# sair-lab/localization

Hardware: AMD Instinct MI355X
Metric: localization updates/sec (8-anchor UWB, batch=65k) (higher is better)
Workload: dtype f64

## Files before the change

include/localization_amd.h:

```cpp
#ifndef LOCALIZATION_AMD_H
#define LOCALIZATION_AMD_H

#include <stddef.h>
#include <stdint.h>

#ifdef __cplusplus
extern "C" {
#endif

#define LOC_ABI_VERSION 4

typedef enum loc_status {
    LOC_OK = 0,
    LOC_ERR_INVALID = -1,
    LOC_ERR_NO_DEVICE = -2,
    LOC_ERR_HIP = -3,
    LOC_ERR_UNKNOWN_NODE = -4,
    LOC_ERR_UNSUPPORTED = -5,
    LOC_ERR_SINGULAR = -6
} loc_status;

enum { LOC_JAC_ANALYTIC = 0, LOC_JAC_NUMERIC_G2O = 1 };

const char* loc_last_error(void);
int32_t loc_abi_version(void);
int32_t loc_device_count(void);

typedef struct loc_shard {
    int32_t rank, world;
    int32_t device;
    int32_t reserved;
    int64_t lo, hi;
} loc_shard;
int loc_shard_bounds(int64_t total, int32_t rank, int32_t world, int64_t* lo, int64_t* hi);
int loc_shard_plan(int64_t total, int32_t world, int32_t devices_per_node, loc_shard* out);

typedef struct loc_snapshot loc_snapshot;

typedef struct loc_snapshot_params {
    int32_t maximum_iteration;
    double distance_outlier;
    int32_t gate_warmup_epochs;
    int32_t jacobian;
    int32_t lanes_per_instance;
    int32_t block_threads;
} loc_snapshot_params;

void loc_snapshot_default_params(loc_snapshot_params* p);

int loc_snapshot_create(loc_snapshot** out, int32_t device, int64_t batch, int32_t n_anchors,
                        const double* anchors_xyz_host, const loc_snapshot_params* params);
int loc_snapshot_destroy(loc_snapshot* s);

int64_t loc_snapshot_batch(const loc_snapshot* s);
int32_t loc_snapshot_anchor_groups(const loc_snapshot* s);
int32_t loc_snapshot_lanes_per_instance(const loc_snapshot* s);
size_t loc_snapshot_range_floats(const loc_snapshot* s, int32_t epochs);

int loc_snapshot_set_positions(loc_snapshot* s, const double* pos_soa_host);
int loc_snapshot_get_positions(loc_snapshot* s, double* pos_soa_host);
void* loc_snapshot_positions_device(loc_snapshot* s);
int64_t loc_snapshot_epochs_done(const loc_snapshot* s);
int loc_snapshot_set_epochs_done(loc_snapshot* s, int64_t epochs);

int loc_snapshot_pack_ranges_host(const loc_snapshot* s, int32_t epochs, const float* src_kmb, float* dst_tiles,
                                  float pad_value);

int loc_snapshot_solve_device(loc_snapshot* s, int32_t epochs, const float* dist_dev, const float* err_dev,
                              double* out_pos_dev, double* out_chi2_dev, uint8_t* out_trials_dev,
                              void* hip_stream);

int loc_snapshot_solve_host(loc_snapshot* s, int32_t epochs, const float* dist_tiles_host,
                            const float* err_tiles_host, double* out_pos_host, double* out_chi2_host,
                            uint8_t* out_trials_host);

int loc_snapshot_solve_host_kmb(loc_snapshot* s, int32_t epochs, const float* dist_kmb_host, const float* err_kmb_host,
                                double* out_pos_host, double* out_chi2_host, uint8_t* out_trials_host);

// ... 178 lines not shown
```

localization_amd/_lib.py:

```python
import ctypes as C
import os

_HERE = os.path.dirname(os.path.abspath(__file__))
_SO = os.environ.get("LOCALIZATION_AMD_LIB") or os.path.join(_HERE, "liblocalization_amd.so")
_LIB = None

LOC_OK = 0
LOC_ERR_NO_DEVICE = -2
JAC_ANALYTIC = 0
JAC_NUMERIC_G2O = 1


class LocalizationAmdError(RuntimeError):
    def __init__(self, code, msg):
        super().__init__(f"localization_amd error {code}: {msg}")
        self.code = code


class SnapshotParams(C.Structure):
    _fields_ = [("maximum_iteration", C.c_int32), ("distance_outlier", C.c_double), ("gate_warmup_epochs", C.c_int32), ("jacobian", C.c_int32),
                ("lanes_per_instance", C.c_int32), ("block_threads", C.c_int32)]


class FusionParams(C.Structure):
    _fields_ = [("maximum_iteration", C.c_int32), ("distance_outlier", C.c_double), ("gate_warmup_epochs", C.c_int32),
                ("antenna_offset", C.c_double * 3), ("block_threads", C.c_int32), ("jacobian", C.c_int32)]


def library_path():
    return _SO


EXPORTED_SYMBOLS = [
    "loc_last_error", "loc_abi_version", "loc_device_count", "loc_shard_bounds", "loc_shard_plan",
    "loc_snapshot_default_params", "loc_snapshot_create", "loc_snapshot_destroy", "loc_snapshot_batch",
    "loc_snapshot_anchor_groups", "loc_snapshot_lanes_per_instance", "loc_snapshot_range_floats",
    "loc_snapshot_set_positions", "loc_snapshot_get_positions", "loc_snapshot_positions_device",
    "loc_snapshot_epochs_done", "loc_snapshot_set_epochs_done",
    "loc_snapshot_pack_ranges_host", "loc_snapshot_solve_device", "loc_snapshot_solve_host",
    "loc_snapshot_solve_host_kmb", "loc_snapshot_solve_device_cov", "loc_snapshot_solve_host_kmb_cov", "loc_host_alloc", "loc_host_free",
    "loc_snapshot_timing_begin", "loc_snapshot_timing_end",
    "loc_window_create", "loc_window_destroy", "loc_window_set_anchors", "loc_window_lds_bytes", "loc_window_solve_host",
    "loc_window_last_kernel_ms", "loc_window_set_endpoint1_offsets", "loc_window_set_prior_information", "loc_window_set_jacobian", "loc_window_set_ordering", "loc_window_set_chain_threshold", "loc_window_last_kernel_kind", "loc_window_set_option", "loc_window_last_host_timing", "loc_window_upload",
    "loc_window_solve_resident", "loc_window_download", "loc_window_poses_device", "loc_window_result_device",
    "loc_window_timing_begin", "loc_window_timing_end",
    "loc_window_covariance_host", "loc_window_covariance_resident", "loc_window_last_covariance_ms", "loc_window_covariance_plan",
    "loc_window_marginal_prior_host", "loc_window_joint_covariance_host", "loc_window_joint_covariance_resident", "loc_window_joint_covariance_plan",
    "loc_window_slide_resident", "loc_window_slide_resident_dev", "loc_window_download_tables",
    "loc_node_default_config", "loc_node_create", "loc_node_destroy", "loc_node_add_range", "loc_node_add_imu",
    "loc_node_add_pose", "loc_node_add_twist", "loc_node_add_lidar", "loc_node_add_rl_range", "loc_node_solve", "loc_node_get_path",
    "loc_node_number_measurements", "loc_node_last_timing", "loc_node_last_kernel_kind", "loc_node_flush_tail", "loc_node_set_deferred", "loc_node_solve_pending", "loc_nodes_solve_batch",
    "loc_nodes_release_batch_cache",
    "loc_fusion_default_params", "loc_fusion_create", "loc_fusion_destroy", "loc_fusion_set_poses", "loc_fusion_get_poses",
    "loc_fusion_solve_device", "loc_fusion_solve_host", "loc_fusion_solve_host_kmb", "loc_fusion_last_kernel_ms", "loc_fusion_timing_begin", "loc_fusion_timing_end",
# ... 198 lines not shown
```

localization_amd/csrc/capi.cpp:

```cpp
#include <algorithm>
#include <cmath>
#include <cstdio>
#include <cstring>
#include <new>
#include <string>
#include <vector>

#include "capi_host.h"
#include "snapshot_kernel.h"

static thread_local std::string g_last_error;

int locamd_fail(int code, const char* what) {
    g_last_error = what ? what : "";
    return code;
}
int locamd_fail_hip(hipError_t e, const char* where) {
    g_last_error = std::string(where) + ": " + hipGetErrorString(e);
    return LOC_ERR_HIP;
}

struct loc_snapshot {
    int device = 0;
    long long B = 0;
// ... 24 lines not shown
}

int loc_shard_bounds(int64_t total, int32_t rank, int32_t world, int64_t* lo, int64_t* hi) {
    if (total < 0 || world <= 0 || rank < 0 || rank >= world || !lo || !hi) return locamd_fail(LOC_ERR_INVALID, "loc_shard_bounds arguments");
    const int64_t per = (total + world - 1) / world;
    const int64_t a = rank * per < total ? rank * per : total;
    *lo = a;
    *hi = a + per < total ? a + per : total;
    return LOC_OK;
}

int loc_shard_plan(int64_t total, int32_t world, int32_t devices_per_node, loc_shard* out) {
    if (total < 0 || world <= 0 || !out) return locamd_fail(LOC_ERR_INVALID, "loc_shard_plan arguments");
    if (devices_per_node <= 0) {
        devices_per_node = loc_device_count();
        if (devices_per_node <= 0) return locamd_fail(LOC_ERR_NO_DEVICE, "no HIP device visible: pass devices_per_node explicitly");
    }
    for (int32_t r = 0; r < world; ++r) {
        out[r].rank = r; out[r].world = world; out[r].device = r % devices_per_node; out[r].reserved = 0;
        const int rc = loc_shard_bounds(total, r, world, &out[r].lo, &out[r].hi);
        if (rc != LOC_OK) return rc;
    }
    return LOC_OK;
}

void loc_snapshot_default_params(loc_snapshot_params* p) {
    if (!p) return;
    p->maximum_iteration = 20;
    p->distance_outlier = 1.0;
    p->gate_warmup_epochs = 1;
    p->jacobian = LOC_JAC_NUMERIC_G2O;
    p->lanes_per_instance = 0;
    p->block_threads = 0;
}

int loc_snapshot_create(loc_snapshot** out, int32_t device, int64_t batch, int32_t n_anchors,
                        const double* anchors_xyz_host, const loc_snapshot_params* params) {
    if (!out) return locamd_fail(LOC_ERR_INVALID, "out is NULL");
    *out = nullptr;
    if (batch <= 0 || n_anchors <= 0 || !anchors_xyz_host) return locamd_fail(LOC_ERR_INVALID, "batch/anchors");
    int ndev = 0;
    if (hipGetDeviceCount(&ndev) != hipSuccess || ndev <= 0)
        return locamd_fail(LOC_ERR_NO_DEVICE, "no HIP device visible: localization_amd has no CPU fallback");
    if (device < 0 || device >= ndev) return locamd_fail(LOC_ERR_INVALID, "device index out of range");
    loc_snapshot_params prm;
    if (params) prm = *params; else loc_snapshot_default_params(&prm);
    if (prm.jacobian != LOC_JAC_ANALYTIC && prm.jacobian != LOC_JAC_NUMERIC_G2O) return locamd_fail(LOC_ERR_INVALID, "jacobian mode");
    const int M4 = (n_anchors + 3) / 4;
    const int M_PAD = 4 * M4;
    if (M_PAD > 16) return locamd_fail(LOC_ERR_UNSUPPORTED, "more than 16 anchors per tag");
    int lpi = prm.lanes_per_instance;
    if (lpi == 0) lpi = (M_PAD == 16) ? 2 : 1;
    if (!locamd::snapshot_supported(M_PAD, lpi)) return locamd_fail(LOC_ERR_UNSUPPORTED, "lanes_per_instance for this anchor count");
    if (prm.block_threads == 0) prm.block_threads = 256;
    if (prm.gate_warmup_epochs < 0) return locamd_fail(LOC_ERR_INVALID, "gate_warmup_epochs");
    if (prm.block_threads % 64 || prm.block_threads > 256 || prm.block_threads < 64) return locamd_fail(LOC_ERR_INVALID, "block_threads");

    LOC_HIP(hipSetDevice(device));
    loc_snapshot* s = new (std::nothrow) loc_snapshot();
    if (!s) return locamd_fail(LOC_ERR_INVALID, "out of host memory");
    s->device = device; s->B = batch; s->M = n_anchors; s->M4 = M4; s->M_PAD = M_PAD; s->lpi = lpi; s->prm = prm;
    std::vector<double> anch((size_t)M_PAD * 3, 0.0);
    std::memcpy(anch.data(), anchors_xyz_host, sizeof(double) * 3 * (size_t)n_anchors);
    hipError_t e;
    if ((e = hipMalloc((void**)&s->d_anchors, anch.size() * sizeof(double))) != hipSuccess ||
        (e = hipMalloc((void**)&s->d_pos, sizeof(double) * 3 * (size_t)batch)) != hipSuccess ||
        (e = hipMemcpy(s->d_anchors, anch.data(), anch.size() * sizeof(double), hipMemcpyHostToDevice)) != hipSuccess ||
        (e = hipMemset(s->d_pos, 0, sizeof(double) * 3 * (size_t)batch)) != hipSuccess ||
        (e = hipStreamCreateWithFlags(&s->own_stream, hipStreamNonBlocking)) != hipSuccess) {
        loc_snapshot_destroy(s);
        return locamd_fail_hip(e, "loc_snapshot_create");
    }
    *out = s;
    return LOC_OK;
}

static int ensure_staging(loc_snapshot* s, int32_t epochs) {
    const size_t nf = loc_snapshot_range_floats(s, epochs), KB = (size_t)epochs * (size_t)s->B;
    LOC_HIP(locamd::grow_buffers(s->staged_epochs, (size_t)epochs, {{s->d_dist, nf * sizeof(float)}, {s->d_err, nf * sizeof(float)},
            {s->d_out_pos, sizeof(double) * 3 * KB}, {s->d_out_chi2, sizeof(double) * KB}, {s->d_out_trials, KB}}));
    return LOC_OK;
}

int loc_snapshot_destroy(loc_snapshot* s) {
    if (!s) return LOC_OK;
    (void)hipSetDevice(s->device);
    s->pipe.destroy();
    s->timer.destroy();
// ... 37 lines not shown
    if (!s || !src || !dst || epochs <= 0) return locamd_fail(LOC_ERR_INVALID, "pack_ranges");
    const size_t B = (size_t)s->B;
    for (int k = 0; k < epochs; ++k)
        for (int g = 0; g < s->M4; ++g)
            for (int j = 0; j < 4; ++j) {
                const int m = 4 * g + j;
                float* d = dst + (((size_t)k * s->M4 + g) * B) * 4 + j;
                if (m < s->M) {
                    const float* sp = src + ((size_t)k * s->M + m) * B;
                    for (size_t b = 0; b < B; ++b) d[4 * b] = sp[b];
                } else {
                    for (size_t b = 0; b < B; ++b) d[4 * b] = pad_value;
                }
            }
    return LOC_OK;
}

}

static int solve_device(loc_snapshot* s, int32_t epochs, const float* dist_dev, const float* err_dev, double* out_pos_dev,
                        double* out_chi2_dev, uint8_t* out_trials_dev, double* cov, int32_t* cov_mask, int32_t* cov_status, void* hip_stream) {
    if (epochs <= 0 || !dist_dev || !err_dev || !out_pos_dev || !out_chi2_dev) return locamd_fail(LOC_ERR_INVALID, "solve arguments");
    if (((uintptr_t)dist_dev | (uintptr_t)err_dev) & 15u) return locamd_fail(LOC_ERR_INVALID, "range tiles must be 16-byte aligned");
    LOC_HIP(hipSetDevice(s->device));
    hipStream_t st = hip_stream ? (hipStream_t)hip_stream : s->own_stream;
    locamd::SnapshotArgs a;
    a.dist = dist_dev; a.err = err_dev; a.pos = s->d_pos; a.out_pos = out_pos_dev; a.out_chi2 = out_chi2_dev;
    a.out_trials = out_trials_dev; a.anchors = s->d_anchors; a.B = s->B; a.K = epochs; a.M4 = s->M4;
    a.iterations = s->prm.maximum_iteration; a.gate = s->prm.distance_outlier;
    {
        long long left = (long long)s->prm.gate_warmup_epochs - s->epochs_done;
        a.gate_from_epoch = left > 0 ? (int)(left > epochs ? epochs : left) : 0;
    }
    LOC_HIP(s->timer.start(st));
    hipError_t e;
    if (!cov) {
        e = locamd::launch_snapshot(a, s->M_PAD, s->lpi, s->prm.jacobian, s->prm.block_threads, st);
    } else {
        locamd::SnapshotCovArgs ca;
        static_cast<locamd::SnapshotArgs&>(ca) = a;
        ca.out_cov = cov; ca.out_cov_mask = cov_mask; ca.out_cov_status = cov_status;
        e = locamd::launch_snapshot_cov(ca, s->M_PAD, s->lpi, s->prm.jacobian, s->prm.block_threads, st);
    }
    if (e != hipSuccess) return locamd_fail_hip(e, "launch_snapshot");
    LOC_HIP(s->timer.stop(st));
    s->epochs_done += epochs;
    return LOC_OK;
}

extern "C" {

int loc_snapshot_solve_device(loc_snapshot* s, int32_t epochs, const float* dist_dev, const float* err_dev,
                              double* out_pos_dev, double* out_chi2_dev, uint8_t* out_trials_dev, void* hip_stream) {
    if (!s) return locamd_fail(LOC_ERR_INVALID, "null handle");
    return solve_device(s, epochs, dist_dev, err_dev, out_pos_dev, out_chi2_dev, out_trials_dev, nullptr, nullptr, nullptr, hip_stream);
}

int loc_snapshot_solve_device_cov(loc_snapshot* s, int32_t epochs, const float* dist_dev, const float* err_dev,
                                  double* out_pos_dev, double* out_chi2_dev, uint8_t* out_trials_dev,
                                  double* out_cov_dev, int32_t* out_cov_mask_dev, int32_t* out_cov_status_dev, void* hip_stream) {
    if (!s) return locamd_fail(LOC_ERR_INVALID, "null handle");
    if (!out_cov_dev || !out_cov_mask_dev || !out_cov_status_dev) return locamd_fail(LOC_ERR_INVALID, "covariance outputs: all three are required");
    return solve_device(s, epochs, dist_dev, err_dev, out_pos_dev, out_chi2_dev, out_trials_dev, out_cov_dev, out_cov_mask_dev,
                        out_cov_status_dev, hip_stream);
}

int loc_snapshot_solve_host(loc_snapshot* s, int32_t epochs, const float* dist_h, const float* err_h,
                            double* out_pos_h, double* out_chi2_h, uint8_t* out_trials_h) {
    if (!s) return locamd_fail(LOC_ERR_INVALID, "null handle");
    if (epochs <= 0 || !dist_h || !err_h || !out_pos_h || !out_chi2_h) return locamd_fail(LOC_ERR_INVALID, "solve arguments");
    LOC_HIP(hipSetDevice(s->device));
    const size_t nf = loc_snapshot_range_floats(s, epochs);
    const size_t B = (size_t)s->B;
    if (int rc = ensure_staging(s, epochs)) return rc;
    LOC_HIP(hipMemcpyAsync(s->d_dist, dist_h, nf * sizeof(float), hipMemcpyHostToDevice, s->own_stream));
// ... 71 lines not shown
```

localization_amd/csrc/snapshot_kernel.h:

```cpp
#pragma once
#include <hip/hip_runtime.h>
#include <stdint.h>

namespace locamd {

struct SnapshotArgs {
    const float* dist;
    const float* err;
    double* pos;
    double* out_pos;
    double* out_chi2;
    uint8_t* out_trials;
    const double* anchors;
    long long B;
    int K;
    int M4;
    int iterations;
    double gate;
    int gate_from_epoch;
};

struct SnapshotCovArgs : SnapshotArgs {
    double* out_cov;
    int32_t* out_cov_mask;
    int32_t* out_cov_status;
};

hipError_t launch_snapshot(const SnapshotArgs& a, int m_pad, int lpi, int jac, int block_threads, hipStream_t stream);
hipError_t launch_snapshot_cov(const SnapshotCovArgs& a, int m_pad, int lpi, int jac, int block_threads, hipStream_t stream);
bool snapshot_supported(int m_pad, int lpi);
hipError_t launch_pack_kmb(const float* src_kmb, float* dst_tiles, long long B, int M, int M4, int K, float pad, hipStream_t stream);

}
```

localization_amd/csrc/snapshot_kernel.hip:

```cpp
#include "snapshot_kernel.h"
#include "device_math.h"
#include "lm_damping.h"
#include "cov_device.h"

#include <float.h>
#include <math.h>

#include <type_traits>

namespace locamd {

namespace {

template <int CTRL>
__device__ __forceinline__ double dpp_move(double v) {
    int lo = __double2loint(v), hi = __double2hiint(v);
    lo = __builtin_amdgcn_update_dpp(0, lo, CTRL, 0xF, 0xF, false);
    hi = __builtin_amdgcn_update_dpp(0, hi, CTRL, 0xF, 0xF, false);
    return __hiloint2double(hi, lo);
}
constexpr int DPP_QUAD_XOR1 = 0xB1;
constexpr int DPP_QUAD_XOR2 = 0x4E;
constexpr int DPP_ROW_HALF_MIRROR = 0x141;

template <int LPI>
__device__ __forceinline__ double group_sum(double v) {
    if constexpr (LPI >= 2) v += dpp_move<DPP_QUAD_XOR1>(v);
    if constexpr (LPI >= 4) v += dpp_move<DPP_QUAD_XOR2>(v);
    if constexpr (LPI >= 8) v += dpp_move<DPP_ROW_HALF_MIRROR>(v);
    return v;
}
template <int LPI>
__device__ __forceinline__ double group_prod(double v) {
    if constexpr (LPI >= 2) v *= dpp_move<DPP_QUAD_XOR1>(v);
    if constexpr (LPI >= 4) v *= dpp_move<DPP_QUAD_XOR2>(v);
    if constexpr (LPI >= 8) v *= dpp_move<DPP_ROW_HALF_MIRROR>(v);
    return v;
}

struct System {
    double h00, h01, h02, h11, h12, h22;
    double b0, b1, b2;
    double rchi;
    double chi;
};

#pragma clang fp contract(off)
__device__ __forceinline__ double range_norm_plain(double dx, double dy, double dz) {
    return sqrt_ieee_unscaled(dx * dx + dy * dy + dz * dz);
}
__device__ __forceinline__ double range_sq_plain(double dx, double dy, double dz) { return dx * dx + dy * dy + dz * dz; }
#pragma clang fp contract(fast)

template <int LPI, int APL, int JAC>
__device__ __forceinline__ System evaluate(const double px, const double py, const double pz,
                                           const double (&ax)[APL], const double (&ay)[APL], const double (&az)[APL],
                                           const double (&d)[APL], double (&w)[APL], const double gate) {
    System s = {0, 0, 0, 0, 0, 0, 0, 0, 0, 0, 0};
    double prod = 1.0;
    int kexp = 0;
#pragma unroll
    for (int j = 0; j < APL; ++j) {
        const double dx = px - ax[j], dy = py - ay[j], dz = pz - az[j];
        double n, jx, jy, jz;
        if constexpr (JAC == 0) {
            const double n2 = fmax(dx * dx + dy * dy + dz * dz, 1e-300);
            double inv;
            sqrt_and_rsqrt_fast(n2, n, inv);
            jx = -dx * inv; jy = -dy * inv; jz = -dz * inv;
        } else {
            constexpr double delta = 1e-9;
            constexpr double scalar = 1.0 / (2 * delta);
            const double x0 = range_sq_plain(dx, dy, dz);
            double h0, c0;
            n = sqrt_ieee_unscaled_raw(x0, h0, c0);
            const double xp = (px + delta) - ax[j], xm = (px - delta) - ax[j];
            const double yp = (py + delta) - ay[j], ym = (py - delta) - ay[j];
            const double zp = (pz + delta) - az[j], zm = (pz - delta) - az[j];
            if (x0 >= 1e-5 && x0 < 1e300) {
                jx = scalar * ((d[j] - sqrt_ieee_near_c(range_sq_plain(xp, dy, dz), n, h0, c0)) - (d[j] - sqrt_ieee_near_c(range_sq_plain(xm, dy, dz), n, h0, c0)));
                jy = scalar * ((d[j] - sqrt_ieee_near_c(range_sq_plain(dx, yp, dz), n, h0, c0)) - (d[j] - sqrt_ieee_near_c(range_sq_plain(dx, ym, dz), n, h0, c0)));
                jz = scalar * ((d[j] - sqrt_ieee_near_c(range_sq_plain(dx, dy, zp), n, h0, c0)) - (d[j] - sqrt_ieee_near_c(range_sq_plain(dx, dy, zm), n, h0, c0)));
            } else {
                n = (x0 == 0.0 || x0 == __builtin_inf()) ? x0 : n;
                jx = scalar * ((d[j] - range_norm_plain(xp, dy, dz)) - (d[j] - range_norm_plain(xm, dy, dz)));
                jy = scalar * ((d[j] - range_norm_plain(dx, yp, dz)) - (d[j] - range_norm_plain(dx, ym, dz)));
                jz = scalar * ((d[j] - range_norm_plain(dx, dy, zp)) - (d[j] - range_norm_plain(dx, dy, zm)));
            }
        }
        const double e = d[j] - n;
// ... 61 lines not shown
    } else if constexpr (APL == 2) {
        const long long idx = ((k * a.M4 + m0 / 4) * B + inst) * 2 + (m0 % 4) / 2;
        const float2 dv = reinterpret_cast<const float2*>(a.dist)[idx];
        const float2 sv = reinterpret_cast<const float2*>(a.err)[idx];
        df[0] = dv.x; df[1] = dv.y; sf[0] = sv.x; sf[1] = sv.y;
    } else {
        static_assert(APL == 1 || APL == 2 || APL % 4 == 0, "anchors per lane");
        const long long idx = ((k * a.M4 + m0 / 4) * B + inst) * 4 + (m0 % 4);
        df[0] = a.dist[idx]; sf[0] = a.err[idx];
    }
}
template <int APL>
__device__ __forceinline__ void ingest(const float (&df)[APL], const float (&sf)[APL], double (&d)[APL], double (&w)[APL]) {
#pragma unroll
    for (int j = 0; j < APL; ++j) {
        const double dd = (double)df[j], ss = (double)sf[j];
        const bool valid = (ss > 0.0) && (ss < DBL_MAX) && (fabs(dd) < DBL_MAX);
        const double cov = valid ? ss * ss : 1.0;
        const double mask = valid ? 1.0 : 0.0;
        d[j] = valid ? dd : 0.0;
        w[j] = fast_rcp(cov) * mask;
    }
}

template <int APL> struct SnapshotLds {
    static constexpr int NEXT_BYTES = APL * 256 * 16;
    static constexpr int RAW_BYTES = (APL % 4 == 0) ? (2 * (APL / 4) * 256 * 16) : 0;
    static constexpr int BYTES = NEXT_BYTES + RAW_BYTES;
};

typedef __attribute__((address_space(3))) void* lds_void_ptr;
typedef const __attribute__((address_space(1))) void* glb_void_ptr;

template <int LPI, int APL, int JAC, bool COV>
__global__ void __launch_bounds__(256) snapshot_lm_kernel(const std::conditional_t<COV, SnapshotCovArgs, SnapshotArgs> a) {
    __shared__ __attribute__((aligned(16))) char lds_bytes[SnapshotLds<APL>::BYTES];
    double2* const s_next = reinterpret_cast<double2*>(lds_bytes);
    float4* const s_raw = reinterpret_cast<float4*>(lds_bytes + SnapshotLds<APL>::NEXT_BYTES);
    const int tib = threadIdx.x;
    const long long tid = (long long)blockIdx.x * blockDim.x + tib;
    const long long inst = tid / LPI;
    const int g = (int)(tid % LPI);
    const long long B = a.B;
    const int K = a.K;
    const bool live = (inst < B) && K > 0;
    const long long ld_inst = live ? inst : 0;
    bool exhausted = !live;

    double ax[APL], ay[APL], az[APL];
    const int m0 = g * APL;
#pragma unroll
    for (int j = 0; j < APL; ++j) {
        ax[j] = a.anchors[(m0 + j) * 3 + 0];
        ay[j] = a.anchors[(m0 + j) * 3 + 1];
        az[j] = a.anchors[(m0 + j) * 3 + 2];
    }

    auto put_next = [&](const double (&dd)[APL], const double (&ww)[APL]) {
#pragma unroll
        for (int j = 0; j < APL; ++j) s_next[j * 256 + tib] = make_double2(dd[j], ww[j]);
    };
    auto take_next = [&](double (&dd)[APL], double (&ww)[APL]) {
        typedef double v2f64 __attribute__((ext_vector_type(2)));
        const unsigned addr = (unsigned)(unsigned long long)(s_next + tib);
        v2f64 v[APL];
#pragma unroll
        for (int j = 0; j < APL; ++j) asm volatile("ds_read_b128 %0, %1 offset:%2" : "=v"(v[j]) : "v"(addr), "n"(j * 4096));
        if constexpr (APL == 8) {
            asm volatile("s_waitcnt lgkmcnt(0)" : "+v"(v[0]), "+v"(v[1]), "+v"(v[2]), "+v"(v[3]), "+v"(v[4]), "+v"(v[5]), "+v"(v[6]), "+v"(v[7]) :: "memory");
        } else {
#pragma unroll
            for (int j = 0; j < APL; ++j) asm volatile("s_waitcnt lgkmcnt(0)" : "+v"(v[j]) :: "memory");
        }
#pragma unroll
        for (int j = 0; j < APL; ++j) { dd[j] = v[j].x; ww[j] = v[j].y; }
    };
    auto prefetch = [&](int ke) {
        if constexpr (APL % 4 == 0) {
            const int wave_base = (tib / 64) * 64;
#pragma unroll
            for (int q4 = 0; q4 < APL / 4; ++q4) {
                const long long idx = ((long long)ke * a.M4 + (m0 / 4 + q4)) * B + ld_inst;
                __builtin_amdgcn_global_load_lds((glb_void_ptr)(reinterpret_cast<const float4*>(a.dist) + idx),
                                                 (lds_void_ptr)(s_raw + q4 * 256 + wave_base), 16, 0, 0);
                __builtin_amdgcn_global_load_lds((glb_void_ptr)(reinterpret_cast<const float4*>(a.err) + idx),
                                                 (lds_void_ptr)(s_raw + (APL / 4 + q4) * 256 + wave_base), 16, 0, 0);
            }
        }
// ... 17 lines not shown

    double px = 0, py = 0, pz = 0;
    double d[APL], w[APL];
    if (live) { px = a.pos[0 * B + inst]; py = a.pos[1 * B + inst]; pz = a.pos[2 * B + inst]; }
    {
        float df0[APL], sf0[APL];
        load_epoch<APL>(a, 0, m0, ld_inst, df0, sf0);
        ingest<APL>(df0, sf0, d, w);
        if (K > 1) {
            double dn[APL], wn[APL];
            load_epoch<APL>(a, 1, m0, ld_inst, df0, sf0);
            ingest<APL>(df0, sf0, dn, wn);
            put_next(dn, wn);
        }
        if (K > 2) prefetch(2);
    }
    asm volatile("" : "+v"(px), "+v"(py), "+v"(pz));

    System cur = {1, 0, 0, 1, 0, 1, 0, 0, 0, 0, 0};
    double cur_chi = 0, last_chi = 0, lambda = 1.0, ni = 2.0;
    int c = 0;
    int k = 0;
    int it = 0, q = 0, trials = 0;
    bool init = true;
    bool waiting = false;

    while (__any(!exhausted)) {
        const bool active = !exhausted && !waiting;
        double x0, x1, x2;
        const bool ok2 = solve3(cur, lambda, x0, x1, x2) && !init;
        if (!ok2) { x0 = 0.0; x1 = 0.0; x2 = 0.0; }
        const double tx = px + x0, ty = py + x1, tz = pz + x2;
        const bool gate_now = active && init && (a.gate > 0.0) && (k >= a.gate_from_epoch);
        const System tr = evaluate<LPI, APL, JAC>(tx, ty, tz, ax, ay, az, d, w, gate_now ? a.gate : DBL_MAX);

        const bool first = active && init;
        const bool lm = active && !init;
        const double temp_chi = ok2 ? tr.rchi : DBL_MAX;
        double scale = x0 * __builtin_fma(lambda, x0, cur.b0) + x1 * __builtin_fma(lambda, x1, cur.b1) +
                       x2 * __builtin_fma(lambda, x2, cur.b2);
        scale += lm_scale_eps;
        const double rho = (cur_chi - temp_chi) * fast_rcp(scale);
        const bool accept = lm && (rho > 0.0) && (fabs(temp_chi) < DBL_MAX) && ok2;
        if (first || accept) {
            cur = tr;
            cur_chi = tr.rchi;
            px = tx; py = ty; pz = tz;
        }
        const double lam_acc = lm_lambda_accepted(lambda, rho);
        const double lam_first = lm_tau * fmax(fabs(tr.h00), fmax(fabs(tr.h11), fabs(tr.h22)));
        lambda = first ? lam_first : (accept ? lam_acc : (lm ? lambda * ni : lambda));
        ni = (first || accept) ? 2.0 : (lm ? ni * 2.0 : ni);
        last_chi = active ? tr.chi : last_chi;
        trials = first ? 0 : trials + (lm ? 1 : 0);
        q = first ? 0 : q + (lm ? 1 : 0);
        const bool end_iter = lm && !((rho < 0.0) && (q < lm_max_trials));
        it = first ? 0 : it + (end_iter ? 1 : 0);
        const bool finished = (first && ((a.iterations <= 0) || !((tr.h00 + tr.h11 + tr.h22) > 0.0))) ||
                              (end_iter && ((q == lm_max_trials) || (rho == 0.0) || (it >= a.iterations)));
        q = end_iter ? 0 : q;
        init = active ? false : init;

        if (__any(finished)) {
            if (finished) {
                if (g == 0) {
                    a.out_pos[((long long)k * 3 + 0) * B + inst] = px;
                    a.out_pos[((long long)k * 3 + 1) * B + inst] = py;
// ... 12 lines not shown
                }
                if (k + 1 >= K) {
                    exhausted = true;
                    if (g == 0) { a.pos[0 * B + inst] = px; a.pos[1 * B + inst] = py; a.pos[2 * B + inst] = pz; }
                } else if (k == c) {
                    take_next(d, w);
                    k = c + 1;
                    init = true;
                } else {
                    waiting = true;
                }
            }
        }
        if (!__any(!exhausted && k == c)) {
            ++c;
            if (c + 1 < K) {
                double dn[APL], wn[APL];
                consume(c + 1, dn, wn);
                put_next(dn, wn);
                asm volatile("" ::: "memory");
                if (c + 2 < K) prefetch(c + 2);
                if (waiting) {
#pragma unroll
                    for (int j = 0; j < APL; ++j) { d[j] = dn[j]; w[j] = wn[j]; }
                    k = c + 1;
                    init = true;
                    waiting = false;
                }
            }
        }
    }
}

template <int LPI, int APL, int JAC, bool COV, class Args>
hipError_t launch_one(const Args& a, int block_threads, hipStream_t stream) {
    const long long lanes = a.B * LPI;
    const long long blocks = (lanes + block_threads - 1) / block_threads;
    if (blocks <= 0 || blocks > 0x7fffffffLL) return hipErrorInvalidValue;
    hipLaunchKernelGGL((snapshot_lm_kernel<LPI, APL, JAC, COV>), dim3((unsigned)blocks), dim3((unsigned)block_threads), 0, stream, a);
    return hipGetLastError();
}

template <int LPI, int APL, bool COV, class Args>
hipError_t launch_jac(const Args& a, int jac, int block_threads, hipStream_t stream) {
    return jac == 0 ? launch_one<LPI, APL, 0, COV>(a, block_threads, stream) : launch_one<LPI, APL, 1, COV>(a, block_threads, stream);
}

template <bool COV, class Args>
hipError_t launch_mapping(const Args& a, int m_pad, int lpi, int jac, int block_threads, hipStream_t stream) {
    if (!snapshot_supported(m_pad, lpi)) return hipErrorInvalidValue;
    if (block_threads <= 0) block_threads = 256;
    if (block_threads % 64 || block_threads > 256) return hipErrorInvalidValue;
    switch (m_pad * 100 + lpi) {
        case 401: return launch_jac<1, 4, COV>(a, jac, block_threads, stream);
        case 402: return launch_jac<2, 2, COV>(a, jac, block_threads, stream);
        case 404: return launch_jac<4, 1, COV>(a, jac, block_threads, stream);
        case 801: return launch_jac<1, 8, COV>(a, jac, block_threads, stream);
        case 802: return launch_jac<2, 4, COV>(a, jac, block_threads, stream);
        case 804: return launch_jac<4, 2, COV>(a, jac, block_threads, stream);
        case 808: return launch_jac<8, 1, COV>(a, jac, block_threads, stream);
        case 1201: return launch_jac<1, 12, COV>(a, jac, block_threads, stream);
        case 1601: return launch_jac<1, 16, COV>(a, jac, block_threads, stream);
        case 1602: return launch_jac<2, 8, COV>(a, jac, block_threads, stream);
        case 1604: return launch_jac<4, 4, COV>(a, jac, block_threads, stream);
        case 1608: return launch_jac<8, 2, COV>(a, jac, block_threads, stream);
        default: return hipErrorInvalidValue;
    }
}

}

namespace {
__global__ void __launch_bounds__(256) pack_kmb_kernel(const float* __restrict__ src, float4* __restrict__ dst, long long B, int M, int M4,
                                                       long long total, float pad) {
    const long long i = (long long)blockIdx.x * 256 + threadIdx.x;
    if (i >= total) return;
    const long long b = i % B, kg = i / B;
    const int g = (int)(kg % M4);
    const long long k = kg / M4;
    const float* row = src + (k * M + 4 * g) * B + b;
    float4 v;
    v.x = 4 * g + 0 < M ? row[0] : pad;
    v.y = 4 * g + 1 < M ? row[B] : pad;
    v.z = 4 * g + 2 < M ? row[2 * B] : pad;
    v.w = 4 * g + 3 < M ? row[3 * B] : pad;
    dst[i] = v;
}
}

hipError_t launch_pack_kmb(const float* src_kmb, float* dst_tiles, long long B, int M, int M4, int K, float pad, hipStream_t stream) {
    const long long total = (long long)K * M4 * B;
    if (total <= 0 || M <= 0 || M > 4 * M4) return hipErrorInvalidValue;
    const long long blocks = (total + 255) / 256;
    if (blocks > 0x7fffffffLL) return hipErrorInvalidValue;
    hipLaunchKernelGGL(pack_kmb_kernel, dim3((unsigned)blocks), dim3(256), 0, stream, src_kmb, reinterpret_cast<float4*>(dst_tiles), B, M, M4, total, pad);
    return hipGetLastError();
}

bool snapshot_supported(int m_pad, int lpi) {
    if (lpi != 1 && lpi != 2 && lpi != 4 && lpi != 8) return false;
    if (m_pad != 4 && m_pad != 8 && m_pad != 12 && m_pad != 16) return false;
    if (m_pad % lpi) return false;
    const int apl = m_pad / lpi;
    if (!(apl == 1 || apl == 2 || apl % 4 == 0)) return false;
    if (m_pad == 12 && lpi != 1) return false;
    return true;
}

hipError_t launch_snapshot(const SnapshotArgs& a, int m_pad, int lpi, int jac, int block_threads, hipStream_t stream) {
    return launch_mapping<false>(a, m_pad, lpi, jac, block_threads, stream);
}

hipError_t launch_snapshot_cov(const SnapshotCovArgs& a, int m_pad, int lpi, int jac, int block_threads, hipStream_t stream) {
    if (!a.out_cov || !a.out_cov_mask || !a.out_cov_status) return hipErrorInvalidValue;
    return launch_mapping<true>(a, m_pad, lpi, jac, block_threads, stream);
}

}
```

localization_amd/snapshot.py:

```python
import ctypes as C

import numpy as np

from . import _lib
from ._lib import SnapshotParams, check, lib


def pack_ranges(x_kmb, pad_value=0.0):
    x = np.ascontiguousarray(x_kmb, dtype=np.float32)
    K, M, B = x.shape
    M4 = (M + 3) // 4
    out = np.full((K, M4 * 4, B), pad_value, dtype=np.float32)
    out[:, :M, :] = x
    return np.ascontiguousarray(out.reshape(K, M4, 4, B).transpose(0, 1, 3, 2))


def unpack_ranges(tiles, M):
    t = np.asarray(tiles)
    K, M4, B, _ = t.shape
    return np.ascontiguousarray(t.transpose(0, 1, 3, 2).reshape(K, M4 * 4, B)[:, :M, :])


class SnapshotSolver(_lib.EpochSolver):
    _prefix = "loc_snapshot"

    def __init__(self, anchors, batch, maximum_iteration=10, distance_outlier=1.0, jacobian="numeric",
                 lanes_per_instance=0, block_threads=0, device=0, gate_warmup_epochs=1):
        import torch
        self.torch = torch
        L = lib()
        if L.loc_device_count() <= 0 or not torch.cuda.is_available():
            raise _lib.LocalizationAmdError(_lib.LOC_ERR_NO_DEVICE,
                                            "no HIP device visible: localization_amd has no CPU fallback")
        anchors = np.ascontiguousarray(anchors, dtype=np.float64)
        assert anchors.ndim == 2 and anchors.shape[1] == 3
        self.M = anchors.shape[0]
        self.B = int(batch)
        self.device = int(device)
        self.dev = torch.device("cuda", self.device)
        prm = SnapshotParams()
        L.loc_snapshot_default_params(C.byref(prm))
        prm.maximum_iteration = int(maximum_iteration)
        prm.distance_outlier = float(distance_outlier)
        prm.gate_warmup_epochs = int(gate_warmup_epochs)
        prm.jacobian = {"analytic": _lib.JAC_ANALYTIC, "numeric": _lib.JAC_NUMERIC_G2O,
                        "numeric_g2o": _lib.JAC_NUMERIC_G2O}[jacobian]
        prm.lanes_per_instance = int(lanes_per_instance)
        prm.block_threads = int(block_threads)
        h = C.c_void_p()
        check(L.loc_snapshot_create(C.byref(h), self.device, self.B, self.M,
                                    anchors.ctypes.data_as(C.POINTER(C.c_double)), C.byref(prm)))
        self.h = h
        self.L = L
        self.M4 = L.loc_snapshot_anchor_groups(h)
        self.lanes_per_instance = L.loc_snapshot_lanes_per_instance(h)

    def set_positions(self, pos_3b):
        p = np.ascontiguousarray(pos_3b, dtype=np.float64)
        assert p.shape == (3, self.B)
        check(self.L.loc_snapshot_set_positions(self.h, p.ctypes.data_as(C.POINTER(C.c_double))))

    def get_positions(self):
        p = np.zeros((3, self.B), dtype=np.float64)
        check(self.L.loc_snapshot_get_positions(self.h, p.ctypes.data_as(C.POINTER(C.c_double))))
        return p

    def to_device_tiles(self, x_kmb, pad_value=0.0):
        return self.torch.from_numpy(pack_ranges(x_kmb, pad_value)).to(self.dev)

    def alloc_outputs(self, K, trials=True, covariance=False):
        return self._device_outputs(K, 3, 6, trials, covariance)

    def solve_device(self, dist_tiles, err_tiles, out_pos, out_chi2, out_trials=None, out_cov=None, out_cov_mask=None, out_cov_status=None):
        t = self.torch
        K = dist_tiles.shape[0]
        assert tuple(dist_tiles.shape) == (K, self.M4, self.B, 4) and dist_tiles.dtype == t.float32
        assert tuple(err_tiles.shape) == tuple(dist_tiles.shape) and err_tiles.dtype == t.float32
        assert dist_tiles.is_contiguous() and err_tiles.is_contiguous()
        assert tuple(out_pos.shape) == (K, 3, self.B) and out_pos.dtype == t.float64 and out_pos.is_contiguous()
        assert tuple(out_chi2.shape) == (K, self.B) and out_chi2.dtype == t.float64 and out_chi2.is_contiguous()
        if out_trials is not None:
# ... 34 lines not shown
```

Measured before the change: 1.996 billion.

## Add cooperative wave tail that spreads per-edge work of few active tags across lanes

Adds a cooperative evaluation path for the 8-anchor, one-lane-per-tag kernel. When a wavefront has at most 8 still-active tags, those tags publish their state to LDS, each of the 64 lanes computes one (tag, edge) term, and the owning lane reduces the terms back. The goal is to cut the divergent long tail where a few unconverged tags keep a whole wave busy running serial 8-edge numeric Jacobians. In exchange it adds LDS per wave, a ballot plus wave barriers on every iteration, and extra code that may raise register pressure. It is on by default for the numeric Jacobian.

Result: no change. 1.997 billion, median of 4 (+0.1%).

```diff
diff --git a/include/localization_amd.h b/include/localization_amd.h
--- a/include/localization_amd.h
+++ b/include/localization_amd.h
@@ -44,6 +44,7 @@
     int32_t jacobian;
     int32_t lanes_per_instance;
     int32_t block_threads;
+    int32_t cooperative_tail;
 } loc_snapshot_params;
 
 void loc_snapshot_default_params(loc_snapshot_params* p);
diff --git a/localization_amd/_lib.py b/localization_amd/_lib.py
--- a/localization_amd/_lib.py
+++ b/localization_amd/_lib.py
@@ -19,7 +19,7 @@
 
 class SnapshotParams(C.Structure):
     _fields_ = [("maximum_iteration", C.c_int32), ("distance_outlier", C.c_double), ("gate_warmup_epochs", C.c_int32), ("jacobian", C.c_int32),
-                ("lanes_per_instance", C.c_int32), ("block_threads", C.c_int32)]
+                ("lanes_per_instance", C.c_int32), ("block_threads", C.c_int32), ("cooperative_tail", C.c_int32)]
 
 
 class FusionParams(C.Structure):
diff --git a/localization_amd/csrc/capi.cpp b/localization_amd/csrc/capi.cpp
--- a/localization_amd/csrc/capi.cpp
+++ b/localization_amd/csrc/capi.cpp
@@ -80,6 +80,7 @@
     p->jacobian = LOC_JAC_NUMERIC_G2O;
     p->lanes_per_instance = 0;
     p->block_threads = 0;
+    p->cooperative_tail = 0;
 }
 
 int loc_snapshot_create(loc_snapshot** out, int32_t device, int64_t batch, int32_t n_anchors,
@@ -102,6 +103,7 @@
     if (!locamd::snapshot_supported(M_PAD, lpi)) return locamd_fail(LOC_ERR_UNSUPPORTED, "lanes_per_instance for this anchor count");
     if (prm.block_threads == 0) prm.block_threads = 256;
     if (prm.gate_warmup_epochs < 0) return locamd_fail(LOC_ERR_INVALID, "gate_warmup_epochs");
+    if (prm.cooperative_tail < -1 || prm.cooperative_tail > 1) return locamd_fail(LOC_ERR_INVALID, "cooperative_tail");
     if (prm.block_threads % 64 || prm.block_threads > 256 || prm.block_threads < 64) return locamd_fail(LOC_ERR_INVALID, "block_threads");
 
     LOC_HIP(hipSetDevice(device));
@@ -205,15 +207,16 @@
         long long left = (long long)s->prm.gate_warmup_epochs - s->epochs_done;
         a.gate_from_epoch = left > 0 ? (int)(left > epochs ? epochs : left) : 0;
     }
+    const bool tail = s->prm.cooperative_tail == 1 || (s->prm.cooperative_tail == 0 && s->prm.jacobian == LOC_JAC_NUMERIC_G2O);
     LOC_HIP(s->timer.start(st));
     hipError_t e;
     if (!cov) {
-        e = locamd::launch_snapshot(a, s->M_PAD, s->lpi, s->prm.jacobian, s->prm.block_threads, st);
+        e = locamd::launch_snapshot(a, s->M_PAD, s->lpi, s->prm.jacobian, s->prm.block_threads, tail, st);
     } else {
         locamd::SnapshotCovArgs ca;
         static_cast<locamd::SnapshotArgs&>(ca) = a;
         ca.out_cov = cov; ca.out_cov_mask = cov_mask; ca.out_cov_status = cov_status;
-        e = locamd::launch_snapshot_cov(ca, s->M_PAD, s->lpi, s->prm.jacobian, s->prm.block_threads, st);
+        e = locamd::launch_snapshot_cov(ca, s->M_PAD, s->lpi, s->prm.jacobian, s->prm.block_threads, tail, st);
     }
     if (e != hipSuccess) return locamd_fail_hip(e, "launch_snapshot");
     LOC_HIP(s->timer.stop(st));
diff --git a/localization_amd/csrc/snapshot_kernel.h b/localization_amd/csrc/snapshot_kernel.h
--- a/localization_amd/csrc/snapshot_kernel.h
+++ b/localization_amd/csrc/snapshot_kernel.h
@@ -26,8 +26,8 @@
     int32_t* out_cov_status;
 };
 
-hipError_t launch_snapshot(const SnapshotArgs& a, int m_pad, int lpi, int jac, int block_threads, hipStream_t stream);
-hipError_t launch_snapshot_cov(const SnapshotCovArgs& a, int m_pad, int lpi, int jac, int block_threads, hipStream_t stream);
+hipError_t launch_snapshot(const SnapshotArgs& a, int m_pad, int lpi, int jac, int block_threads, bool cooperative_tail, hipStream_t stream);
+hipError_t launch_snapshot_cov(const SnapshotCovArgs& a, int m_pad, int lpi, int jac, int block_threads, bool cooperative_tail, hipStream_t stream);
 bool snapshot_supported(int m_pad, int lpi);
 hipError_t launch_pack_kmb(const float* src_kmb, float* dst_tiles, long long B, int M, int M4, int K, float pad, hipStream_t stream);
 
diff --git a/localization_amd/csrc/snapshot_kernel.hip b/localization_amd/csrc/snapshot_kernel.hip
--- a/localization_amd/csrc/snapshot_kernel.hip
+++ b/localization_amd/csrc/snapshot_kernel.hip
@@ -50,12 +50,152 @@
     return sqrt_ieee_unscaled(dx * dx + dy * dy + dz * dz);
 }
 __device__ __forceinline__ double range_sq_plain(double dx, double dy, double dz) { return dx * dx + dy * dy + dz * dz; }
+__device__ __forceinline__ double mul_plain(double a, double b) { return a * b; }
+__device__ __forceinline__ double add_plain(double a, double b) { return a + b; }
 #pragma clang fp contract(fast)
 
-template <int LPI, int APL, int JAC>
+#ifndef LOCAMD_SNAPSHOT_COOP_MAX_TAGS
+#define LOCAMD_SNAPSHOT_COOP_MAX_TAGS 8
+#endif
+constexpr int COOP_APL = 8;
+constexpr int COOP_MAX_TAGS = LOCAMD_SNAPSHOT_COOP_MAX_TAGS;
+static_assert(COOP_MAX_TAGS >= 1 && COOP_MAX_TAGS * COOP_APL <= 64, "one lane per (tag, edge) pair");
+
+struct EdgeTerms {
+    double jx, jy, jz;
+    double e, w, chi;
+    double aux;
+    double wjx, wjy, wjz;
+};
+constexpr int EDGE_TERMS = 10;
+
+template <int JAC>
+__device__ __forceinline__ EdgeTerms edge_terms(const double px, const double py, const double pz, const double ax, const double ay,
+                                                const double az, const double d, const double w, const double gate) {
+    EdgeTerms t;
+    const double dx = px - ax, dy = py - ay, dz = pz - az;
+    double n;
+    if constexpr (JAC == 0) {
+        const double n2 = fmax(__builtin_fma(dz, dz, __builtin_fma(dy, dy, dx * dx)), 1e-300);
+        double inv;
+        sqrt_and_rsqrt_fast(n2, n, inv);
+        t.jx = -dx * inv; t.jy = -dy * inv; t.jz = -dz * inv;
+    } else {
+        constexpr double delta = 1e-9;
+        constexpr double scalar = 1.0 / (2 * delta);
+        const double x0 = range_sq_plain(dx, dy, dz);
+        double h0, c0;
+        n = sqrt_ieee_unscaled_raw(x0, h0, c0);
+        const double xp = (px + delta) - ax, xm = (px - delta) - ax;
+        const double yp = (py + delta) - ay, ym = (py - delta) - ay;
+        const double zp = (pz + delta) - az, zm = (pz - delta) - az;
+        if (x0 >= 1e-5 && x0 < 1e300) {
+            t.jx = scalar * ((d - sqrt_ieee_near_c(range_sq_plain(xp, dy, dz), n, h0, c0)) - (d - sqrt_ieee_near_c(range_sq_plain(xm, dy, dz), n, h0, c0)));
+            t.jy = scalar * ((d - sqrt_ieee_near_c(range_sq_plain(dx, yp, dz), n, h0, c0)) - (d - sqrt_ieee_near_c(range_sq_plain(dx, ym, dz), n, h0, c0)));
+            t.jz = scalar * ((d - sqrt_ieee_near_c(range_sq_plain(dx, dy, zp), n, h0, c0)) - (d - sqrt_ieee_near_c(range_sq_plain(dx, dy, zm), n, h0, c0)));
+        } else {
+            n = (x0 == 0.0 || x0 == __builtin_inf()) ? x0 : n;
+            t.jx = scalar * ((d - range_norm_plain(xp, dy, dz)) - (d - range_norm_plain(xm, dy, dz)));
+            t.jy = scalar * ((d - range_norm_plain(dx, yp, dz)) - (d - range_norm_plain(dx, ym, dz)));
+            t.jz = scalar * ((d - range_norm_plain(dx, dy, zp)) - (d - range_norm_plain(dx, dy, zm)));
+        }
+    }
+    t.e = d - n;
+    t.w = (fabs(t.e) > gate) ? 0.0 : w;
+    const double we = t.w * t.e;
+    t.chi = mul_plain(t.e, we);
+    t.aux = __builtin_fma(t.e, we, 1.0);
+    const double rho1 = fast_rcp_1nr(t.aux);
+    const double wr = rho1 * t.w;
+    t.wjx = wr * t.jx; t.wjy = wr * t.jy; t.wjz = wr * t.jz;
+    return t;
+}
+
+__device__ __forceinline__ void accumulate_edge(System& s, double& prod, int& kexp, const EdgeTerms& t, const bool take_exp) {
+    s.h00 = __builtin_fma(t.wjx, t.jx, s.h00); s.h01 = __builtin_fma(t.wjx, t.jy, s.h01); s.h02 = __builtin_fma(t.wjx, t.jz, s.h02);
+    s.h11 = __builtin_fma(t.wjy, t.jy, s.h11); s.h12 = __builtin_fma(t.wjy, t.jz, s.h12); s.h22 = __builtin_fma(t.wjz, t.jz, s.h22);
+    s.b0 = __builtin_fma(-t.wjx, t.e, s.b0); s.b1 = __builtin_fma(-t.wjy, t.e, s.b1); s.b2 = __builtin_fma(-t.wjz, t.e, s.b2);
+    prod *= t.aux;
+    if (take_exp) { kexp = __builtin_amdgcn_frexp_exp(prod); prod = __builtin_amdgcn_frexp_mant(prod); }
+    s.chi = add_plain(s.chi, t.chi);
+}
+
+template <int JAC>
+__device__ __forceinline__ System evaluate_edges(const double px, const double py, const double pz, const double (&ax)[COOP_APL],
+                                                 const double (&ay)[COOP_APL], const double (&az)[COOP_APL], const double (&d)[COOP_APL],
+                                                 double (&w)[COOP_APL], const double gate) {
+    System s = {0, 0, 0, 0, 0, 0, 0, 0, 0, 0, 0};
+    double prod = 1.0;
+    int kexp = 0;
+#pragma unroll
+    for (int j = 0; j < COOP_APL; ++j) {
+        const EdgeTerms t = edge_terms<JAC>(px, py, pz, ax[j], ay[j], az[j], d[j], w[j], gate);
+        w[j] = t.w;
+        accumulate_edge(s, prod, kexp, t, j == 3);
+    }
+    s.rchi = fast_log_ge1_scaled(prod, kexp);
+    return s;
+}
+
+struct CoopLds {
+    double anchor[COOP_APL][3];
+    double pub[COOP_MAX_TAGS][4 + 2 * COOP_APL];
+    double terms[EDGE_TERMS][64];
+};
+
+template <int JAC>
+__device__ __forceinline__ System evaluate_coop(CoopLds& L, const unsigned long long ballot, const bool active, const int lane,
+                                                const double px, const double py, const double pz, const double (&d)[COOP_APL],
+                                                double (&w)[COOP_APL], const double gate) {
+    const int n_slots = __popcll(ballot);
+    const int rank = (int)__builtin_amdgcn_mbcnt_hi((unsigned)(ballot >> 32), __builtin_amdgcn_mbcnt_lo((unsigned)ballot, 0u));
+    if (active) {
+        double* const p = L.pub[rank];
+        p[0] = px; p[1] = py; p[2] = pz; p[3] = gate;
+#pragma unroll
+        for (int j = 0; j < COOP_APL; ++j) { p[4 + j] = d[j]; p[4 + COOP_APL + j] = w[j]; }
+    }
+    __builtin_amdgcn_wave_barrier();
+    const int slot = lane / COOP_APL, edge = lane % COOP_APL;
+    if (slot < n_slots) {
+        const double* const p = L.pub[slot];
+        const EdgeTerms t = edge_terms<JAC>(p[0], p[1], p[2], L.anchor[edge][0], L.anchor[edge][1], L.anchor[edge][2], p[4 + edge],
+                                            p[4 + COOP_APL + edge], p[3]);
+        L.terms[0][lane] = t.jx; L.terms[1][lane] = t.jy; L.terms[2][lane] = t.jz;
+        L.terms[3][lane] = t.e; L.terms[4][lane] = t.w; L.terms[5][lane] = t.chi; L.terms[6][lane] = t.aux;
+        L.terms[7][lane] = t.wjx; L.terms[8][lane] = t.wjy; L.terms[9][lane] = t.wjz;
+    }
+    __builtin_amdgcn_wave_barrier();
+    System s = {0, 0, 0, 0, 0, 0, 0, 0, 0, 0, 0};
+    if (active) {
+        double prod = 1.0;
+        int kexp = 0;
+#pragma unroll
+        for (int j = 0; j < COOP_APL; ++j) {
+            const int l = rank * COOP_APL + j;
+            EdgeTerms t;
+            t.jx = L.terms[0][l]; t.jy = L.terms[1][l]; t.jz = L.terms[2][l];
+            t.e = L.terms[3][l]; t.w = L.terms[4][l]; t.chi = L.terms[5][l]; t.aux = L.terms[6][l];
+            t.wjx = L.terms[7][l]; t.wjy = L.terms[8][l]; t.wjz = L.terms[9][l];
+            w[j] = t.w;
+            accumulate_edge(s, prod, kexp, t, j == 3);
+        }
+        s.rchi = fast_log_ge1_scaled(prod, kexp);
+    }
+    __builtin_amdgcn_wave_barrier();
+    return s;
+}
+
+template <int LPI, int APL, int JAC, bool COOP>
 __device__ __forceinline__ System evaluate(const double px, const double py, const double pz,
                                            const double (&ax)[APL], const double (&ay)[APL], const double (&az)[APL],
-                                           const double (&d)[APL], double (&w)[APL], const double gate) {
+                                           const double (&d)[APL], double (&w)[APL], const double gate,
+                                           [[maybe_unused]] CoopLds* coop, [[maybe_unused]] const bool active, [[maybe_unused]] const int lane) {
+    if constexpr (COOP) {
+        const unsigned long long ballot = __ballot(active);
+        if (__popcll(ballot) <= COOP_MAX_TAGS) return evaluate_coop<JAC>(*coop, ballot, active, lane, px, py, pz, d, w, gate);
+        return evaluate_edges<JAC>(px, py, pz, ax, ay, az, d, w, gate);
+    }
     System s = {0, 0, 0, 0, 0, 0, 0, 0, 0, 0, 0};
     double prod = 1.0;
     int kexp = 0;
@@ -183,9 +323,10 @@
 typedef __attribute__((address_space(3))) void* lds_void_ptr;
 typedef const __attribute__((address_space(1))) void* glb_void_ptr;
 
-template <int LPI, int APL, int JAC, bool COV>
+template <int LPI, int APL, int JAC, bool COV, bool COOP = false>
 __global__ void __launch_bounds__(256) snapshot_lm_kernel(const std::conditional_t<COV, SnapshotCovArgs, SnapshotArgs> a) {
-    __shared__ __attribute__((aligned(16))) char lds_bytes[SnapshotLds<APL>::BYTES];
+    static_assert(!COOP || (LPI == 1 && APL == COOP_APL), "the cooperative tail is for one lane per tag and 8 anchors");
+    __shared__ __attribute__((aligned(16))) char lds_bytes[SnapshotLds<APL>::BYTES + (COOP ? 4 * sizeof(CoopLds) : 0)];
     double2* const s_next = reinterpret_cast<double2*>(lds_bytes);
     float4* const s_raw = reinterpret_cast<float4*>(lds_bytes + SnapshotLds<APL>::NEXT_BYTES);
     const int tib = threadIdx.x;
@@ -205,6 +346,11 @@
         ax[j] = a.anchors[(m0 + j) * 3 + 0];
         ay[j] = a.anchors[(m0 + j) * 3 + 1];
         az[j] = a.anchors[(m0 + j) * 3 + 2];
+    }
+    [[maybe_unused]] CoopLds* coop = nullptr;
+    if constexpr (COOP) {
+        coop = reinterpret_cast<CoopLds*>(lds_bytes + SnapshotLds<APL>::BYTES) + tib / 64;
+        if (tib % 64 < COOP_APL * 3) (&coop->anchor[0][0])[tib % 64] = a.anchors[tib % 64];
     }
 
     auto put_next = [&](const double (&dd)[APL], const double (&ww)[APL]) {
@@ -288,7 +434,7 @@
         if (!ok2) { x0 = 0.0; x1 = 0.0; x2 = 0.0; }
         const double tx = px + x0, ty = py + x1, tz = pz + x2;
         const bool gate_now = active && init && (a.gate > 0.0) && (k >= a.gate_from_epoch);
-        const System tr = evaluate<LPI, APL, JAC>(tx, ty, tz, ax, ay, az, d, w, gate_now ? a.gate : DBL_MAX);
+        const System tr = evaluate<LPI, APL, JAC, COOP>(tx, ty, tz, ax, ay, az, d, w, gate_now ? a.gate : DBL_MAX, coop, active, tib % 64);
 
         const bool first = active && init;
         const bool lm = active && !init;
@@ -367,22 +513,22 @@
     }
 }
 
-template <int LPI, int APL, int JAC, bool COV, class Args>
+template <int LPI, int APL, int JAC, bool COV, bool COOP, class Args>
 hipError_t launch_one(const Args& a, int block_threads, hipStream_t stream) {
     const long long lanes = a.B * LPI;
     const long long blocks = (lanes + block_threads - 1) / block_threads;
     if (blocks <= 0 || blocks > 0x7fffffffLL) return hipErrorInvalidValue;
-    hipLaunchKernelGGL((snapshot_lm_kernel<LPI, APL, JAC, COV>), dim3((unsigned)blocks), dim3((unsigned)block_threads), 0, stream, a);
+    hipLaunchKernelGGL((snapshot_lm_kernel<LPI, APL, JAC, COV, COOP>), dim3((unsigned)blocks), dim3((unsigned)block_threads), 0, stream, a);
     return hipGetLastError();
 }
 
-template <int LPI, int APL, bool COV, class Args>
+template <int LPI, int APL, bool COV, bool COOP = false, class Args>
 hipError_t launch_jac(const Args& a, int jac, int block_threads, hipStream_t stream) {
-    return jac == 0 ? launch_one<LPI, APL, 0, COV>(a, block_threads, stream) : launch_one<LPI, APL, 1, COV>(a, block_threads, stream);
+    return jac == 0 ? launch_one<LPI, APL, 0, COV, COOP>(a, block_threads, stream) : launch_one<LPI, APL, 1, COV, COOP>(a, block_threads, stream);
 }
 
 template <bool COV, class Args>
-hipError_t launch_mapping(const Args& a, int m_pad, int lpi, int jac, int block_threads, hipStream_t stream) {
+hipError_t launch_mapping(const Args& a, int m_pad, int lpi, int jac, int block_threads, bool cooperative_tail, hipStream_t stream) {
     if (!snapshot_supported(m_pad, lpi)) return hipErrorInvalidValue;
     if (block_threads <= 0) block_threads = 256;
     if (block_threads % 64 || block_threads > 256) return hipErrorInvalidValue;
@@ -390,7 +536,7 @@
         case 401: return launch_jac<1, 4, COV>(a, jac, block_threads, stream);
         case 402: return launch_jac<2, 2, COV>(a, jac, block_threads, stream);
         case 404: return launch_jac<4, 1, COV>(a, jac, block_threads, stream);
-        case 801: return launch_jac<1, 8, COV>(a, jac, block_threads, stream);
+        case 801: return cooperative_tail ? launch_jac<1, 8, COV, true>(a, jac, block_threads, stream) : launch_jac<1, 8, COV>(a, jac, block_threads, stream);
         case 802: return launch_jac<2, 4, COV>(a, jac, block_threads, stream);
         case 804: return launch_jac<4, 2, COV>(a, jac, block_threads, stream);
         case 808: return launch_jac<8, 1, COV>(a, jac, block_threads, stream);
@@ -442,13 +588,13 @@
     return true;
 }
 
-hipError_t launch_snapshot(const SnapshotArgs& a, int m_pad, int lpi, int jac, int block_threads, hipStream_t stream) {
-    return launch_mapping<false>(a, m_pad, lpi, jac, block_threads, stream);
-}
-
-hipError_t launch_snapshot_cov(const SnapshotCovArgs& a, int m_pad, int lpi, int jac, int block_threads, hipStream_t stream) {
+hipError_t launch_snapshot(const SnapshotArgs& a, int m_pad, int lpi, int jac, int block_threads, bool cooperative_tail, hipStream_t stream) {
+    return launch_mapping<false>(a, m_pad, lpi, jac, block_threads, cooperative_tail, stream);
+}
+
+hipError_t launch_snapshot_cov(const SnapshotCovArgs& a, int m_pad, int lpi, int jac, int block_threads, bool cooperative_tail, hipStream_t stream) {
     if (!a.out_cov || !a.out_cov_mask || !a.out_cov_status) return hipErrorInvalidValue;
-    return launch_mapping<true>(a, m_pad, lpi, jac, block_threads, stream);
-}
-
-}
+    return launch_mapping<true>(a, m_pad, lpi, jac, block_threads, cooperative_tail, stream);
+}
+
+}
diff --git a/localization_amd/snapshot.py b/localization_amd/snapshot.py
--- a/localization_amd/snapshot.py
+++ b/localization_amd/snapshot.py
@@ -25,7 +25,7 @@
     _prefix = "loc_snapshot"
 
     def __init__(self, anchors, batch, maximum_iteration=10, distance_outlier=1.0, jacobian="numeric",
-                 lanes_per_instance=0, block_threads=0, device=0, gate_warmup_epochs=1):
+                 lanes_per_instance=0, block_threads=0, device=0, gate_warmup_epochs=1, cooperative_tail=None):
         import torch
         self.torch = torch
         L = lib()
@@ -47,6 +47,7 @@
                         "numeric_g2o": _lib.JAC_NUMERIC_G2O}[jacobian]
         prm.lanes_per_instance = int(lanes_per_instance)
         prm.block_threads = int(block_threads)
+        prm.cooperative_tail = 0 if cooperative_tail is None else (1 if cooperative_tail else -1)
         h = C.c_void_p()
         check(L.loc_snapshot_create(C.byref(h), self.device, self.B, self.M,
                                     anchors.ctypes.data_as(C.POINTER(C.c_double)), C.byref(prm)))
```
